# simonfuhrmann/mve

Measured on NVIDIA H100. Metric: mvs_depth_pixels_per_second, higher is better.
Workload: dtype f32

## Files before the change

### mve_b200/csrc/b200mvs.cu

```cuda
#include "../../include/b200mvs.h"
#include "patch_opt.cuh"
#include "patch_warp.cuh"
#include "patch_thread.cuh"
#include "pset_device.cuh"
#include "device_buffer.cuh"
#include "plan_device.cuh"

#include <algorithm>
#include <cmath>
#include <cstdarg>
#include <cstddef>
#include <cstdio>
#include <cstring>
#include <cstdlib>
#include <functional>
#include <map>
#include <chrono>
#include <ctime>
#include <mutex>
#include <string>
#include <thread>
#include <atomic>
#include <vector>

// ... 619 lines not shown
}

__host__ __device__ inline int slots_to_ids(const int* gview, int n_global, unsigned word, int32_t ids[4])
{
    int n = 0;
#pragma unroll
    for (int k = 0; k < 4; ++k) {
        const unsigned sl = (word >> (8 * k)) & 0xFF;
        ids[k] = sl < (unsigned)n_global ? gview[sl] : -1;
        n += ids[k] >= 0;
    }
    return n;
}

__global__ void k_slots_to_ids(const JobParams job, int32_t* __restrict__ out, bool aligned16)
{
    const size_t p = (size_t)blockIdx.x * blockDim.x + threadIdx.x;
    if (p >= (size_t)job.W * job.H) return;
    int32_t ids[4];
    slots_to_ids(job.gview, job.n_global, __ldg(job.slots + p), ids);
    int32_t* o = out + 4 * p;
    if (aligned16) *reinterpret_cast<int4*>(o) = make_int4(ids[0], ids[1], ids[2], ids[3]);
    else { o[0] = ids[0]; o[1] = ids[1]; o[2] = ids[2]; o[3] = ids[3]; }
}

#ifndef OPT_MIN_BLOCKS
#define OPT_MIN_BLOCKS 1
#endif
constexpr int OPT_WARPS = OPT_TPB / 32;
using PatchT = b200mvs::PatchW;
using PatchT1 = b200mvs::PatchT;
constexpr size_t OPT_LUT_BYTES = sizeof(float) * (256 * LUT_STRIDE);
constexpr size_t OPT_SMEM_BYTES = OPT_LUT_BYTES + (size_t)OPT_TPB * sizeof(PatchT1) + PatchT1::MT_BYTES;
static_assert(OPT_SMEM_BYTES + 8 + 1024 <= 196 * 1024, "the patch kernels' shared memory must stay within the 196 KB carve-out");
__device__ __forceinline__ PatchT1& thread_patch(float* smem)
{
    return reinterpret_cast<PatchT1*>(reinterpret_cast<unsigned char*>(smem) + OPT_LUT_BYTES)[threadIdx.x];
}

__device__ __forceinline__ Entry load_entry(const Entry* p)
{
    const int4 a = __ldcg(reinterpret_cast<const int4*>(p));
    const int4 b = __ldcg(reinterpret_cast<const int4*>(p) + 1);
    Entry e;
    e.xy = a.x; e.jobdir = a.y; e.conf = __int_as_float(a.z); e.depth = __int_as_float(a.w);
    e.dzI = __int_as_float(b.x); e.dzJ = __int_as_float(b.y); e.slots = (unsigned)b.z; e.pad = b.w;
    return e;
}

__device__ __forceinline__ PatchIn patch_in(const Entry& e)
{
    PatchIn pi;
    pi.x = entry_x(e); pi.y = entry_y(e);
    pi.depth = e.depth; pi.dzI = e.dzI; pi.dzJ = e.dzJ; pi.slots = e.slots;
    return pi;
}

__device__ __forceinline__ unsigned long long global_timer_ns()
{
    unsigned long long t;
    asm volatile("mov.u64 %0, %%globaltimer;" : "=l"(t));
    return t;
}

__device__ __forceinline__ void optimise_entries(PatchT& p, const Entry* list, PatchOut* res, unsigned long long n,
                                                 unsigned long long* ticket, const JobParams* jobs, unsigned long long* counters)
{
// ... 35 lines not shown
            const unsigned long long w = base + (unsigned long long)__popc(act & ((1u << lane) - 1u));
            if (w >= n) break;
            idx = w;
            const Entry e = load_entry(&list[w]);
            p.begin(&jobs[entry_job(e)], patch_in(e));
            have = true;
            ++opts;
        }
        if (p.step()) {
            PatchOut po;
            p.finish(po);
            res[idx] = po;
            have = false;
        }
    }
    if (opts) {
        atomicAdd(&counters[C_SETS], (unsigned long long)p.n_sets);
        atomicAdd(&counters[C_OPTS], (unsigned long long)opts);
        p.n_sets = 0u;
    }
}

#ifndef OPT_THREAD_MIN
#define OPT_THREAD_MIN 8192
#endif

__global__ void __launch_bounds__(OPT_TPB, OPT_MIN_BLOCKS)
k_optimize(const Entry* __restrict__ in, PatchOut* __restrict__ out, int n, int mode,
           const DevSettings* __restrict__ st, const JobParams* __restrict__ jobs, const ViewParams* __restrict__ views,
           const float* __restrict__ g_lut, unsigned long long* counters)
{
    extern __shared__ float smem[];
    for (int i = threadIdx.x; i < 256 * LUT_STRIDE; i += blockDim.x) smem[i] = g_lut[i / LUT_STRIDE];
    __syncthreads();
    if (mode == 2 || (mode == 0 && n >= OPT_THREAD_MIN)) {
        PatchT1& p = thread_patch(smem);
        bind_thread(p, st, views, smem, (int)threadIdx.x);
        optimise_entries_t(p, in, out, (unsigned long long)n, &counters[C_TICKET], jobs, counters);
    } else {
        PatchT p;
        bind_thread(p, st, views, smem, (int)threadIdx.x);
        optimise_entries(p, in, out, (unsigned long long)n, &counters[C_TICKET], jobs, counters);
    }
}

__device__ __forceinline__ unsigned long long entry_key(const Entry& e)
{
    return ((unsigned long long)__float_as_uint(e.conf) << 8) | (unsigned long long)(7 - entry_dir(e));
}

struct FrontierParams {
    Entry* list[2];
    Entry* run;
    Entry* run2;
    unsigned* tile_cnt;
    unsigned long long* tile_off;
    long long n_tiles;
    PatchOut* res;
    unsigned char* written;
    unsigned long long cap;
    int n_seeds, n_jobs;
    const DevSettings* st;
    const JobParams* jobs;
    const ViewParams* views;
    const float* lut;
    unsigned long long* counters;
// ... 135 lines not shown
        const int j = entry_job(e);
        const JobParams& J = P.jobs[j];
        const int x = entry_x(e), y = entry_y(e);
        const int nx[4] = {x - 1, x + 1, x, x};
        const int ny[4] = {y, y, y - 1, y + 1};
#pragma unroll
        for (int d = 0; d < 4; ++d) {
            const float c = __ldcg(&J.conf[ny[d] * J.W + nx[d]]);
            if (c < r.conf - 0.05f || c == 0.f) push_entry(P, 1 - p, child_entry(pack_xy(nx[d], ny[d]), j, d, r));
        }
    }
}

__device__ __forceinline__ bool end_round(FrontierCtl* ctl, unsigned long long n_cur, const HostMirror* host)
{
    ctl->rounds += 1ull;
    if (n_cur > ctl->peak) ctl->peak = n_cur;
    return host->cancel != 0;
}

__global__ void k_frontier_resume(const FrontierParams P)
{
    FrontierCtl* const ctl = P.ctl;
    const size_t gtid = (size_t)blockIdx.x * blockDim.x + threadIdx.x, gthreads = (size_t)gridDim.x * blockDim.x;
    push_neighbours(P, ctl->resume_p, ctl->resume_sorted ? P.run2 : P.run, ctl->resume_nrun, gtid, gthreads);
    if (gtid == 0) ctl->stop = end_round(ctl, ctl->resume_ncur, P.host) ? ST_CANCELLED : ST_RUN;
}

__global__ void __launch_bounds__(OPT_TPB, OPT_MIN_BLOCKS)
k_frontier(const FrontierParams P)
{
    extern __shared__ float smem[];
    for (int i = threadIdx.x; i < 256 * LUT_STRIDE; i += blockDim.x) smem[i] = P.lut[i / LUT_STRIDE];
    __syncthreads();
    const int lane = threadIdx.x & 31;
    const size_t gtid = (size_t)blockIdx.x * blockDim.x + threadIdx.x, gthreads = (size_t)gridDim.x * blockDim.x;
    FrontierCtl* const ctl = P.ctl;
    unsigned long long* const cnt = P.counters;
    unsigned long long* const filled = cnt + C_NUM;
    const bool lead = blockIdx.x == 0 && threadIdx.x == 0;
    const bool thresholded = P.band_bins > 0 || P.topk > 0;
    unsigned long long t_prev = lead ? global_timer_ns() : 0ull;
    unsigned long long n_bar = 0ull;
#define PHASE_END(ph) do { grid_barrier(&ctl->bar); ++n_bar; if (lead) { const unsigned long long t_ = global_timer_ns(); ctl->ns[ph] += t_ - t_prev; t_prev = t_; } } while (0)

    int p = P.first_list;
    bool seed_round = P.n_seeds > 0;
    for (;;) {
        unsigned long long n_cur = seed_round ? (unsigned long long)P.n_seeds : __ldcg(&ctl->nlist[p]);
        if (n_cur > P.cap) n_cur = P.cap;
        if (__ldcg(&ctl->stop) != ST_RUN || n_cur == 0ull) break;
        unsigned long long n_run = n_cur;
        if (!seed_round) {
        Entry* const cur = P.list[p];
        if (blockIdx.x == 0) {
            if (threadIdx.x == 0) { P.host->round = ctl->rounds; P.host->queue = n_cur; }
            for (int j = threadIdx.x; j < P.n_jobs; j += blockDim.x) {
                P.host_filled[j] = __ldcg(&filled[j]);
                if (P.host_cancel_job[j]) P.job_cancel[j] = 1;
            }
        }
        for (size_t i = gtid; i < n_cur; i += gthreads) {
            const Entry e = load_entry(&cur[i]);
            const int j = entry_job(e);
            const JobParams& J = P.jobs[j];
            const int idx = pixel_of(J, e);
// ... 1589 lines not shown
```

### mve_b200/csrc/patch_opt.cuh

```cuda
#pragma once
#if defined(B200MVS_HOST_EMU)
#include "simt_emu.h"
#else
#include <cuda_runtime.h>
#endif
#include <stdint.h>
#include <cstddef>

namespace b200mvs {

constexpr int MAX_LEVELS = 12;
constexpr int MAX_GLOBAL = 32;
constexpr int MAX_LOCAL = 4;
constexpr unsigned FULL = 0xffffffffu;
constexpr int NS = 25;
constexpr int CENTER = 12;
constexpr int LUT_REP = 32;
constexpr int LUT_STRIDE = 64;

struct alignas(16) LevelParams {
    float ax, ay, cx, cy;
    int w, h;
    int pitch;
    int pad;
// ... 211 lines not shown
                              ((stage == POST) & ((p.iter + 1) % 5 == 4));
        float cand[MAX_GLOBAL];
        PassOut po = {0.f, 0.f, 0.f, 0.f, 0.f};
        p.pass(a_cand, a_cs, a_ncc, a_normal, cand, po);
        if (stage == LVS_CTOR || stage == LVS_REPL) {
            p.lvs_greedy(cand);
            if (!p.is(F_LVS_OK)) { if (stage == LVS_CTOR) p.pk &= ~F_OPTI; p.set_stage(DONE); return true; }
            p.set_stage((stage == LVS_CTOR) ? CTOR : REPL);
            return false;
        }
        if (!p.is(F_OPTI)) { p.set_stage(DONE); return true; }
        if (stage == POST) {
            const int n = p.nsel();
            const unsigned dfb = (p.pk >> SH_DF) & ((1u << n) - 1u);
            const unsigned tbr = ((p.iter == 14) ? dfb : 0u) | p.low_ncc_mask();
            if (tbr) {
                p.pk |= F_VIEW_REMOVED;
                p.sel_erase_mask(tbr);
                p.pk &= ~F_LVS_OK;
                p.set_stage(LVS_REPL);
                return false;
            }
            if (dfb == 0u) { p.pk |= F_CONVERGED; p.set_stage(DONE); return true; }
            ++p.iter;
        } else if (stage == REPL) {
            ++p.iter;
        }
        while (p.iter < 4 && p.is(F_OPTI)) {
            const bool moved = depth_step(p, po);
            ++p.iter;
            if (moved && p.is(F_OPTI)) { p.set_stage(FIRST); return false; }
        }
        if (!p.is(F_OPTI)) { p.set_stage(DONE); return true; }
        if (!((unsigned)p.iter < p.st->max_iterations && p.is(F_LVS_OK))) { p.set_stage(DONE); return true; }
        const bool normal = (p.iter % 5 == 4) || p.is(F_VIEW_REMOVED);
        p.put(F_NORMAL, normal);
        if (!p.is(F_HAS_NCC) || (normal && !p.is(F_HAS_NORMAL))) { p.set_stage(PRE); return false; }
        p.pk &= ~F_OPTI;
        if (normal) { normal_step(p, po); p.pk &= ~F_VIEW_REMOVED; p.pk |= F_WAS_NORMAL; }
        else { depth_step(p, po); p.pk &= ~F_WAS_NORMAL; }
        if (!p.is(F_OPTI)) { p.set_stage(DONE); return true; }
        p.set_stage(POST);
        return false;
    }
};

}
```

### mve_b200/csrc/patch_thread.cuh

```cuda
#pragma once
#include "patch_opt.cuh"
#if defined(B200MVS_HOST_EMU)
#include <cassert>
#endif

#ifndef OPT_TPB
#define OPT_TPB 384
#endif

namespace b200mvs {

struct alignas(8) SampleOffset { float di, dj; };
#if !defined(B200MVS_HOST_EMU)
__constant__
#endif
static const SampleOffset k_sample_offset[NS] = {
    {-2.f, -2.f}, {-1.f, -2.f}, {0.f, -2.f}, {1.f, -2.f}, {2.f, -2.f},
    {-2.f, -1.f}, {-1.f, -1.f}, {0.f, -1.f}, {1.f, -1.f}, {2.f, -1.f},
    {-2.f,  0.f}, {-1.f,  0.f}, {0.f,  0.f}, {1.f,  0.f}, {2.f,  0.f},
    {-2.f,  1.f}, {-1.f,  1.f}, {0.f,  1.f}, {1.f,  1.f}, {2.f,  1.f},
    {-2.f,  2.f}, {-1.f,  2.f}, {0.f,  2.f}, {1.f,  2.f}, {2.f,  2.f}};

struct PatchT : PatchState {
    const DevSettings* st;
    const ViewParams* views;
#if defined(B200MVS_HOST_EMU)
    const float* lut_tab;
    unsigned lane4;
    unsigned mt_k[NS];
#endif
    const JobParams* job;
    unsigned xy;
    float u0x, u0y, u0z;
    float uax, uay, uaz;
    float ubx, uby, ubz;
    float c0x, c0y, c0z;
    float mx0, mx1, mx2;
    float crx, cry, crz;
    float cpx, cpy, cpz;
    float mfp, inv_mfp;
    float mm, inv_mm, sqrDevX;
    unsigned selp;
    float cs[MAX_LOCAL][3];
    float ncc[MAX_LOCAL];

    __device__ __forceinline__ int sel(int k) const { return (int)((selp >> (8 * k)) & 0xFFu); }
    __device__ __forceinline__ int px() const { return (int)(xy & 0xFFFFu); }
    __device__ __forceinline__ int py() const { return (int)(xy >> 16); }

    template <typename T> static __device__ __forceinline__ T get4(const T (&a)[MAX_LOCAL], int k)
    {
        return k == 0 ? a[0] : (k == 1 ? a[1] : (k == 2 ? a[2] : a[3]));
    }
    template <typename T> static __device__ __forceinline__ void set4(T (&a)[MAX_LOCAL], int k, T v)
    {
#pragma unroll
        for (int i = 0; i < MAX_LOCAL; ++i) if (i == k) a[i] = v;
    }

    __device__ __forceinline__ unsigned lane_offset() const
    {
#if defined(B200MVS_HOST_EMU)
        return lane4;
#else
        return (threadIdx.x & 31u) << 2;
#endif
    }
    __device__ __forceinline__ const float* table() const
    {
#if defined(B200MVS_HOST_EMU)
        return lut_tab;
#else
        extern __shared__ float b200mvs_dyn_smem[];
        return b200mvs_dyn_smem;
#endif
    }

#if defined(B200MVS_HOST_EMU)
    static constexpr unsigned MT_STRIDE = 1u;
#else
    static constexpr unsigned MT_STRIDE = OPT_TPB;
#endif
    static constexpr size_t MT_BYTES = sizeof(unsigned) * NS * OPT_TPB;
    __device__ __forceinline__ unsigned* mt_tab()
    {
#if defined(B200MVS_HOST_EMU)
        return mt_k;
#else
        extern __shared__ float b200mvs_dyn_smem[];
        return reinterpret_cast<unsigned*>(b200mvs_dyn_smem + (256 * LUT_STRIDE + OPT_TPB * (sizeof(PatchT) / sizeof(float)))) + threadIdx.x;
#endif
    }

    __device__ __forceinline__ void sample_ray(float di, float dj, float& ux, float& uy, float& uz, float& inv) const
    {
        ux = u0x + di * uax + dj * ubx;
        uy = u0y + di * uay + dj * uby;
        uz = u0z + di * uaz + dj * ubz;
        inv = rsqrt_fast(ux * ux + uy * uy + uz * uz);
    }

    __device__ __forceinline__ void compute_points()
    {
        bool bad = false;
#pragma unroll 5
        for (int k = 0; k < NS; ++k) {
            const float t = depth + (float)(k % 5 - 2) * dzI + (float)(k / 5 - 2) * dzJ;
            bad |= t <= 0.f;
        }
        if (bad) pk &= ~F_REF_OK;
        cpx = c0x + depth * crx;
        cpy = c0y + depth * cry;
        cpz = c0z + depth * crz;
        const ViewParams* rv = &views[job->ref_view];
        const float z = __ldg(&rv->w2c[8]) * cpx + __ldg(&rv->w2c[9]) * cpy + __ldg(&rv->w2c[10]) * cpz + __ldg(&rv->w2c[11]);
        mfp = z * job->ki0;
        inv_mfp = rcp_fast(mfp);
    }

    __device__ __forceinline__ void init_sampler(int x, int y)
    {
        const float* const lut_tab = table();
        const unsigned lane4 = lane_offset();
        pk &= ~F_REF_OK; mm = 0.f; inv_mm = 0.f; sqrDevX = 0.f;
        mx0 = mx1 = mx2 = 0.f;
        crx = cry = crz = cpx = cpy = cpz = mfp = inv_mfp = 0.f;
        if (x - 2 < 0 || y - 2 < 0 || x + 2 > job->W - 1 || y + 2 > job->H - 1) return;
        {
            const ViewParams* rv = &views[job->ref_view];
            const float r0 = __ldg(&rv->rot[0]), r1 = __ldg(&rv->rot[1]), r2 = __ldg(&rv->rot[2]), r3 = __ldg(&rv->rot[3]), r4 = __ldg(&rv->rot[4]);
            const float r5 = __ldg(&rv->rot[5]), r6 = __ldg(&rv->rot[6]), r7 = __ldg(&rv->rot[7]), r8 = __ldg(&rv->rot[8]);
            const float vx = job->ki0 * ((float)x + 0.5f) + job->ki2, vy = job->ki4 * ((float)y + 0.5f) + job->ki5;
            u0x = r0 * vx + r3 * vy + r6; u0y = r1 * vx + r4 * vy + r7; u0z = r2 * vx + r5 * vy + r8;
            uax = r0 * job->ki0; uay = r1 * job->ki0; uaz = r2 * job->ki0;
            ubx = r3 * job->ki4; uby = r4 * job->ki4; ubz = r5 * job->ki4;
            c0x = __ldg(&rv->campos[0]); c0y = __ldg(&rv->campos[1]); c0z = __ldg(&rv->campos[2]);
            const float inv = rsqrt_fast(u0x * u0x + u0y * u0y + u0z * u0z);
            crx = u0x * inv; cry = u0y * inv; crz = u0z * inv;
        }
        pk |= F_REF_OK;
        unsigned* const mt = mt_tab();
        const uchar4* row = job->ref_img + (size_t)(y - 2) * job->ref_pitch + (x - 2);
        float s0 = 0.f, s1 = 0.f, s2 = 0.f;
#pragma unroll 1
        for (int j = 0; j < 5; ++j) {
#pragma unroll
            for (int i = 0; i < 5; ++i) {
                const unsigned t = reinterpret_cast<const unsigned*>(row)[i];
                s0 += lut_k<0>(lut_tab, lane4, t); s1 += lut_k<1>(lut_tab, lane4, t); s2 += lut_k<2>(lut_tab, lane4, t);
                mt[(5 * j + i) * MT_STRIDE] = t;
            }
            row += job->ref_pitch;
        }
        mm = (s0 + s1 + s2) / (3.f * NS);
        if (mm < 0.01f || mm > 0.99f) { pk &= ~F_REF_OK; return; }
        inv_mm = 1.f / mm;
        mx0 = (s0 * inv_mm) / (float)NS; mx1 = (s1 * inv_mm) / (float)NS; mx2 = (s2 * inv_mm) / (float)NS;
        float dev = 0.f;
#pragma unroll 1
        for (int j = 0; j < 5; ++j) {
#pragma unroll
            for (int i = 0; i < 5; ++i) {
                const unsigned t = mt[(5 * j + i) * MT_STRIDE];
                const float e0 = lut_k<0>(lut_tab, lane4, t) * inv_mm - mx0, e1 = lut_k<1>(lut_tab, lane4, t) * inv_mm - mx1, e2 = lut_k<2>(lut_tab, lane4, t) * inv_mm - mx2;
                dev += e0 * e0 + e1 * e1 + e2 * e2;
            }
        }
        sqrDevX = dev;
        compute_points();
    }

    struct Staged {
        uint4 Q;
        unsigned mt;
        float fx, fy, gx, gy;
    };
    struct Sweep {
        const float* lut;
        unsigned lane4;
        float inv_mm;
        float u0x, u0y, u0z, uax, uay, uaz, ubx, uby, ubz, depth, dzI, dzJ;
        const unsigned* mt;
        float A0x, A0y, A0z, W0x, W0y, W0z, Wax, Way, Waz, Wbx, Wby, Wbz;
        float Lax, Lay, Lcx, Lcy, wm1, hm1, step, dd;
        const uint4* quad;
        unsigned qpitch;
        float pv0, pv1, pv2;
        float c0, c1, c2;
        bool nrm;
// ... 49 lines not shown
            const float omfx = sub_rn(1.f, fx), omfy = sub_rn(1.f, fy), wxy = fma_rn(fy, gx, mul_rn(fx, gy));
            float n[3], d[3];
#pragma unroll
            for (int ch = 0; ch < 3; ++ch) {
                const float x0 = fma_rn(omfx, a[ch], mul_rn(fx, b[ch]));
                const float x3 = fma_rn(omfx, c[ch], mul_rn(fx, e[ch]));
                n[ch] = fma_rn(omfy, x0, mul_rn(fy, x3));
                const float t = fma_rn(gx, sub_rn(b[ch], a[ch]), mul_rn(gy, sub_rn(c[ch], a[ch])));
                d[ch] = mul_rn(fma_rn(wxy, add_rn(sub_rn(sub_rn(a[ch], b[ch]), c[ch]), e[ch]), t), dd);
            }
            const float y0 = sub_rn(n[0], pv0), y1 = sub_rn(n[1], pv1), y2 = sub_rn(n[2], pv2);
            Sya = add_rn(Sya, y0); Syb = add_rn(Syb, y1); Syc = add_rn(Syc, y2);
            Syya = fma_rn(y0, y0, Syya); Syyb = fma_rn(y1, y1, Syyb); Syyc = fma_rn(y2, y2, Syyc);
            Smya = fma_rn(m[0], y0, Smya); Smyb = fma_rn(m[1], y1, Smyb); Smyc = fma_rn(m[2], y2, Smyc);
            Sdma = fma_rn(d[0], m[0], Sdma); Sdmb = fma_rn(d[1], m[1], Sdmb); Sdmc = fma_rn(d[2], m[2], Sdmc);
            Sdna = fma_rn(d[0], n[0], Sdna); Sdnb = fma_rn(d[1], n[1], Sdnb); Sdnc = fma_rn(d[2], n[2], Sdnc);
            Sdda = fma_rn(d[0], d[0], Sdda); Sddb = fma_rn(d[1], d[1], Sddb); Sddc = fma_rn(d[2], d[2], Sddc);
            if (nrm) {
                const float di = k_sample_offset[k].di, dj = k_sample_offset[k].dj;
                const float g0 = mul_rn(c0, d[0]), g1 = mul_rn(c1, d[1]), g2 = mul_rn(c2, d[2]);
                const float q = fma_rn(g2, g2, fma_rn(g0, g0, mul_rn(g1, g1)));
                const float s = fma_rn(g2, fma_rn(-c2, n[2], m[2]), fma_rn(g0, fma_rn(-c0, n[0], m[0]), mul_rn(g1, fma_rn(-c1, n[1], m[1]))));
                const float qi = mul_rn(di, q), qj = mul_rn(dj, q);
                A1 = add_rn(A1, qi); A2 = add_rn(A2, qj); A3 = fma_rn(di, qi, A3); A4 = fma_rn(dj, qi, A4); A5 = fma_rn(dj, qj, A5);
                B1 = fma_rn(di, s, B1); B2 = fma_rn(dj, s, B2);
            }
        }
    };

    __device__ __forceinline__ void pass(bool candidates, bool cs_pending, bool want_ncc, bool want_normal, float* cand, PassOut& po)
    {
        const float* const lut_tab = table();
        const unsigned lane4 = lane_offset();
        const float u0x = this->u0x, u0y = this->u0y, u0z = this->u0z, uax = this->uax, uay = this->uay, uaz = this->uaz;
        const float ubx = this->ubx, uby = this->uby, ubz = this->ubz;
        const float depth = this->depth, dzI = this->dzI, dzJ = this->dzJ;
        const float inv_mm = this->inv_mm;
        const JobParams* const job = this->job;
        float num = 0.f, den = 0.f;
        double D0 = 0.0, D1 = 0.0, D2 = 0.0, D3 = 0.0, D4 = 0.0, D5 = 0.0, E0 = 0.0, E1 = 0.0, E2 = 0.0;
        bool cs_active = cs_pending && st->use_color_scale;
        if (!candidates) pk &= want_ncc ? ~((0xFFu << SH_COL) | (0xFu << SH_DF)) : ~(0xFFu << SH_COL);
        const int count = candidates ? job->n_global : nsel();
        const float pv0 = mx0 * mm, pv1 = mx1 * mm, pv2 = mx2 * mm;
#pragma unroll 1
        for (int k = 0; k < count; ++k) {
            int slot = k;
            if (candidates) { if (!((avail >> k) & 1u)) continue; }
            else slot = sel(k);
            const ViewParams* V = &views[job->gview[slot]];
            ++n_sets;
            float c0 = 1.f, c1 = 1.f, c2 = 1.f;
            if (!candidates) {
                c0 = k == 0 ? cs[0][0] : (k == 1 ? cs[1][0] : (k == 2 ? cs[2][0] : cs[3][0]));
                c1 = k == 0 ? cs[0][1] : (k == 1 ? cs[1][1] : (k == 2 ? cs[2][1] : cs[3][1]));
                c2 = k == 0 ? cs[0][2] : (k == 1 ? cs[1][2] : (k == 2 ? cs[2][2] : cs[3][2]));
            }
            unsigned r = 0u;
            float A0x = 0.f, A0y = 0.f, A0z = 0.f, W0x = 0.f, W0y = 0.f, W0z = 0.f, Wax = 0.f, Way = 0.f, Waz = 0.f, Wbx = 0.f, Wby = 0.f, Wbz = 0.f;
            float Lax = 0.f, Lay = 0.f, Lcx = 0.f, Lcy = 0.f, wm1 = 0.f, hm1 = 0.f, dd = 0.f, step = 0.f;
            int Lpitch = 0;
            const uint4* Lquad = nullptr;
            {
                const float4 wa = __ldg(reinterpret_cast<const float4*>(&V->w2c[0]));
                const float4 wb = __ldg(reinterpret_cast<const float4*>(&V->w2c[4]));
                const float4 wc = __ldg(reinterpret_cast<const float4*>(&V->w2c[8]));
                A0x = wa.x * c0x + wa.y * c0y + wa.z * c0z + wa.w;
                A0y = wb.x * c0x + wb.y * c0y + wb.z * c0z + wb.w;
                A0z = wc.x * c0x + wc.y * c0y + wc.z * c0z + wc.w;
                W0x = wa.x * u0x + wa.y * u0y + wa.z * u0z; W0y = wb.x * u0x + wb.y * u0y + wb.z * u0z; W0z = wc.x * u0x + wc.y * u0y + wc.z * u0z;
                Wax = wa.x * uax + wa.y * uay + wa.z * uaz; Way = wb.x * uax + wb.y * uay + wb.z * uaz; Waz = wc.x * uax + wc.y * uay + wc.z * uaz;
                Wbx = wa.x * ubx + wa.y * uby + wa.z * ubz; Wby = wb.x * ubx + wb.y * uby + wb.z * ubz; Wbz = wc.x * ubx + wc.y * uby + wc.z * ubz;
                const float nz = wc.x * cpx + wc.y * cpy + wc.z * cpz + wc.w;
                const float nfp = nz * __ldg(&V->inv_ax0);
                if (mfp > 0.f && !(nfp <= 0.f)) {
                    const int l = level_of(V, nfp, inv_mfp);
                    const float4 kk = __ldg(reinterpret_cast<const float4*>(&V->lv[l].ax));
                    const int4 g = __ldg(reinterpret_cast<const int4*>(&V->lv[l].w));
                    Lax = kk.x; Lay = kk.y; Lcx = kk.z; Lcy = kk.w; wm1 = (float)(g.x - 1); hm1 = (float)(g.y - 1); Lpitch = g.z;
                    Lquad = reinterpret_cast<const uint4*>(__ldg(reinterpret_cast<const unsigned long long*>(&V->lv[l].quad)));
                    const float inv0 = rsqrt_fast(u0x * u0x + u0y * u0y + u0z * u0z);
                    const float sa = depth * inv0, sb = (depth + 1.f) * inv0;
                    const float hz1 = A0z + sa * W0z, hz2 = A0z + sb * W0z;
                    const float i1 = rcp_fast(hz1), i2 = rcp_fast(hz2);
                    const float ddx = (Lax * (A0x + sb * W0x) + Lcx * hz2) * i2 - (Lax * (A0x + sa * W0x) + Lcx * hz1) * i1;
                    const float ddy = (Lay * (A0y + sb * W0y) + Lcy * hz2) * i2 - (Lay * (A0y + sa * W0y) + Lcy * hz1) * i1;
                    const float dd2 = ddx * ddx + ddy * ddy;
                    dd = dd2 * rsqrt_fast(dd2);
                    step = rcp_fast(dd);
                    r = dd > 0.f ? 3u : 1u;
                }
            }
            const bool need_ncc = candidates || want_ncc;
            const bool cs_view = !candidates && cs_active;
            float nccv = -1.f;
#pragma unroll 1
            for (int rep = 0; rep < 2 && r != 0u; ++rep) {
                const bool second = rep == 1;
                if (second && !(cs_view && want_normal && (r & 2u))) break;
                const bool gn = !candidates && (r & 2u) && (second || !(cs_view && want_normal));
                const bool nrm = gn && want_normal;
                Sweep sw;
                sw.lut = lut_tab; sw.lane4 = lane4; sw.inv_mm = inv_mm;
                sw.u0x = u0x; sw.u0y = u0y; sw.u0z = u0z; sw.uax = uax; sw.uay = uay; sw.uaz = uaz; sw.ubx = ubx; sw.uby = uby; sw.ubz = ubz;
                sw.mt = mt_tab();
                sw.depth = depth; sw.dzI = dzI; sw.dzJ = dzJ;
                sw.A0x = A0x; sw.A0y = A0y; sw.A0z = A0z; sw.W0x = W0x; sw.W0y = W0y; sw.W0z = W0z;
                sw.Wax = Wax; sw.Way = Way; sw.Waz = Waz; sw.Wbx = Wbx; sw.Wby = Wby; sw.Wbz = Wbz;
                sw.Lax = Lax; sw.Lay = Lay; sw.Lcx = Lcx; sw.Lcy = Lcy; sw.wm1 = wm1; sw.hm1 = hm1; sw.step = step; sw.dd = dd;
// ... 24 lines not shown
                    const float sqrDevY = (Syya - Sya * Sya * inv_n) + (Syyb - Syb * Syb * inv_n) + (Syyc - Syc * Syc * inv_n);
                    const float Sen = (Smya - mx0 * Sya) + (Smyb - mx1 * Syb) + (Smyc - mx2 * Syc);
                    const float p = sqrDevX * sqrDevY;
                    nccv = p > 0.f ? Sen * rsqrt_fast(p) : -1.f;
                }
                if (!second && cs_view) {
                    const float Mna = Smya + pv0 * ((float)NS * mx0), Mnb = Smyb + pv1 * ((float)NS * mx1), Mnc = Smyc + pv2 * ((float)NS * mx2);
                    const float Nna = Syya + pv0 * (2.f * Sya + (float)NS * pv0), Nnb = Syyb + pv1 * (2.f * Syb + (float)NS * pv1);
                    const float Nnc = Syyc + pv2 * (2.f * Syc + (float)NS * pv2);
                    float cc[3] = {c0, c1, c2};
                    const float ab[3] = {Mna - c0 * Nna, Mnb - c1 * Nnb, Mnc - c2 * Nnc};
                    const float aa[3] = {Nna, Nnb, Nnc};
                    colour_scale_step(cc, ab, aa);
                    c0 = cc[0]; c1 = cc[1]; c2 = cc[2];
#pragma unroll
                    for (int i = 0; i < MAX_LOCAL; ++i) if (i == k) { cs[i][0] = c0; cs[i][1] = c1; cs[i][2] = c2; }
                }
                if (gn) {
                    const float vn = c0 * (Sdma - c0 * Sdna) + c1 * (Sdmb - c1 * Sdnb) + c2 * (Sdmc - c2 * Sdnc);
                    const float vd = c0 * c0 * Sdda + c1 * c1 * Sddb + c2 * c2 * Sddc;
                    num += vn; den += vd;
                    if (nrm) {
                        D0 += (double)vd; D1 += (double)A1; D2 += (double)A2; D3 += (double)A3; D4 += (double)A4; D5 += (double)A5;
                        E0 += (double)vn; E1 += (double)B1; E2 += (double)B2;
                    }
                }
            }
            if (!candidates) {
                if (r & 1u) pk |= 1u << (SH_COL + k);
                if (r & 2u) pk |= 1u << (SH_DER + k);
                if (cs_active && !(r & 1u)) cs_active = false;
                if (want_ncc) {
                    const float v = (r & 1u) ? nccv : -1.f;
                    if (fabsf(v - get4(ncc, k)) > st->min_refine_diff) pk |= 1u << (SH_DF + k);
                    set4(ncc, k, v);
                }
            } else {
                const float v = (r & 1u) ? nccv : -1.f;
                if (v < st->min_ncc) avail &= ~(1u << k);
                else cand[k] = v;
            }
        }
        if (candidates) return;
        po.num = num; po.den = den;
        put(F_HAS_NORMAL, want_normal);
        put(F_HAS_NCC, want_ncc);
        if (want_normal) {
            const double m[9] = {D0, D1, D2, D1, D3, D4, D2, D4, D5};
            const double det = m[0] * m[4] * m[8] + m[1] * m[5] * m[6] + m[2] * m[3] * m[7]
                             - m[2] * m[4] * m[6] - m[1] * m[3] * m[8] - m[0] * m[5] * m[7];
            put(F_SINGULAR, det == 0.0);
            double inv[9];
            inv[0] = m[4] * m[8] - m[5] * m[7];
            inv[1] = m[2] * m[7] - m[1] * m[8];
            inv[2] = m[1] * m[5] - m[2] * m[4];
            inv[3] = m[5] * m[6] - m[3] * m[8];
            inv[4] = m[0] * m[8] - m[2] * m[6];
            inv[5] = m[2] * m[3] - m[0] * m[5];
            inv[6] = m[3] * m[7] - m[4] * m[6];
            inv[7] = m[1] * m[6] - m[0] * m[7];
            inv[8] = m[0] * m[4] - m[1] * m[3];
#pragma unroll
            for (int q = 0; q < 9; ++q) inv[q] /= det;
            po.nX0 = (float)(inv[0] * E0 + inv[1] * E1 + inv[2] * E2);
            po.nX1 = (float)(inv[3] * E0 + inv[4] * E1 + inv[5] * E2);
            po.nX2 = (float)(inv[6] * E0 + inv[7] * E1 + inv[8] * E2);
        }
    }

    __device__ __forceinline__ void sel_erase_mask(unsigned mask)
    {
        const int n = nsel();
// ... 2 lines not shown
#pragma unroll
        for (int k = 0; k < MAX_LOCAL; ++k) {
            if (k < n && !((mask >> k) & 1u)) {
                const unsigned s8 = (selp >> (8 * k)) & 0xFFu;
                const float a = cs[k][0], b = cs[k][1], c = cs[k][2], v = ncc[k];
                packed = (packed & ~(0xFFu << (8 * cnt))) | (s8 << (8 * cnt));
#pragma unroll
                for (int q = 0; q < MAX_LOCAL; ++q) if (q == cnt) { cs[q][0] = a; cs[q][1] = b; cs[q][2] = c; ncc[q] = v; }
                ++cnt;
            }
        }
        selp = packed;
        set_nsel(cnt);
    }
    __device__ __forceinline__ void sel_insert(int slot, float cs_init)
    {
        const int n = nsel();
        int pos = 0;
#pragma unroll
        for (int k = 0; k < MAX_LOCAL; ++k) if (k < n && sel(k) < slot) ++pos;
#pragma unroll
        for (int q = MAX_LOCAL - 1; q > 0; --q)
            if (q > pos && q <= n) { cs[q][0] = cs[q - 1][0]; cs[q][1] = cs[q - 1][1]; cs[q][2] = cs[q - 1][2]; ncc[q] = ncc[q - 1]; }
#pragma unroll
        for (int q = 0; q < MAX_LOCAL; ++q) if (q == pos) { cs[q][0] = cs[q][1] = cs[q][2] = cs_init; ncc[q] = 0.f; }
        const unsigned low = pos == 0 ? 0u : (selp & (0xFFFFFFFFu >> (32 - 8 * pos)));
        const unsigned high = pos >= 3 ? 0u : ((selp >> (8 * pos)) << (8 * (pos + 1)));
        selp = low | ((unsigned)slot << (8 * pos)) | high;
        set_nsel(n + 1);
    }

    __device__ __forceinline__ void lvs_greedy(const float* cand)
    {
        const unsigned N = st->nr_recon_neighbors;
        const float cs_init = 1.f / mm;
        float rdx = cpx - c0x, rdy = cpy - c0y, rdz = cpz - c0z;
        {
            const float nn = sqrtf(rdx * rdx + rdy * rdy + rdz * rdz);
            rdx /= nn; rdy /= nn; rdz /= nn;
        }
        const int G = job->n_global;
        bool found = true;
        while ((unsigned)nsel() < N && found) {
            found = false;
            float maxScore = 0.f;
            int maxView = 0;
#pragma unroll 1
            for (int c = 0; c < G; ++c) {
                if (!((avail >> c) & 1u)) continue;
                float vdx, vdy, vdz, epx, epy, epz, nfp;
                view_geometry(&views[job->gview[c]], cpx, cpy, cpz, rdx, rdy, rdz, vdx, vdy, vdz, epx, epy, epz, nfp);
                float score = cand[c];
                if (mfp / nfp < 0.5f) score *= 0.01f;
                float dp = clamp1(rdx * vdx + rdy * vdy + rdz * vdz);
                score *= plx_weight(deg_acos(dp));
                const int ns = nsel();
#pragma unroll 1
                for (int k = 0; k < ns; ++k) {
                    float sx, sy, sz, ex, ey, ez, sfp;
                    view_geometry(&views[job->gview[sel(k)]], cpx, cpy, cpz, rdx, rdy, rdz, sx, sy, sz, ex, ey, ez, sfp);
                    lvs_weigh(score, vdx, vdy, vdz, epx, epy, epz, sx, sy, sz, ex, ey, ez, st->min_parallax);
                }
                if (score > maxScore) { maxScore = score; maxView = c; found = true; }
            }
            if (found) {
                sel_insert(maxView, cs_init);
                avail &= ~(1u << maxView);
            }
        }
        if ((unsigned)nsel() == N) pk |= F_LVS_OK;
    }

    __device__ __forceinline__ void begin(const JobParams* j, const PatchIn& in)
    {
        job = j;
        xy = ((unsigned)in.x & 0xFFFFu) | ((unsigned)in.y << 16);
        reset(in);
        u0x = u0y = u0z = uax = uay = uaz = ubx = uby = ubz = c0x = c0y = c0z = 0.f;
        init_sampler(in.x, in.y);
        selp = in.slots;
        int n = 0;
#pragma unroll
        for (int k = 0; k < MAX_LOCAL; ++k) {
            if (sel(k) != 0xFF) n = k + 1;
            cs[k][0] = cs[k][1] = cs[k][2] = 0.f; ncc[k] = 0.f;
        }
        set_nsel(n);
        if (!is(F_REF_OK)) { pk &= ~F_OPTI; return; }
        const unsigned N = st->nr_recon_neighbors;
        if ((unsigned)n == N) pk |= F_LVS_OK;
        else if ((unsigned)n > N) {
            n = 0;
            set_nsel(0);
            selp = 0xFFFFFFFFu;
        }
        avail = job->n_global >= 32 ? FULL : ((1u << job->n_global) - 1u);
#pragma unroll
        for (int k = 0; k < MAX_LOCAL; ++k) if (k < n) avail &= ~(1u << sel(k));
        const float ci = 1.f / mm;
#pragma unroll
        for (int k = 0; k < MAX_LOCAL; ++k) { cs[k][0] = cs[k][1] = cs[k][2] = ci; }
        set_stage(is(F_LVS_OK) ? CTOR : LVS_CTOR);
    }

    __device__ __forceinline__ unsigned low_ncc_mask() const
    {
        const int n = nsel();
        unsigned m = 0u;
#pragma unroll
        for (int k = 0; k < MAX_LOCAL; ++k)
            if (k < n && ncc[k] < st->accept_ncc) m |= 1u << k;
        return m;
    }

    __device__ __forceinline__ bool step() { return auto_step(*this); }

    __device__ __forceinline__ void finish(PatchOut& out)
    {
        finish_state(out);
        const int n = nsel();
        out.slots = n >= 4 ? selp : (selp | (0xFFFFFFFFu << (8 * n)));
        if (!is(F_CONVERGED)) return;
        float mean = 0.f;
#pragma unroll
        for (int k = 0; k < MAX_LOCAL; ++k) if (k < n) mean += ncc[k];
        mean /= (float)n;
        float px[4], py[4], pz[4];
        const float di_[4] = {2.f, -2.f, 0.f, 0.f}, dj_[4] = {0.f, 0.f, -2.f, 2.f};
#pragma unroll
        for (int q = 0; q < 4; ++q) {
            float ux, uy, uz, inv;
            sample_ray(di_[q], dj_[q], ux, uy, uz, inv);
            const float s1 = (depth + di_[q] * dzI + dj_[q] * dzJ) * inv;
            px[q] = c0x + s1 * ux; py[q] = c0y + s1 * uy; pz[q] = c0z + s1 * uz;
        }
        const float ax_ = px[0] - px[1], ay_ = py[0] - py[1], az_ = pz[0] - pz[1];
        const float bx_ = px[2] - px[3], by_ = py[2] - py[3], bz_ = pz[2] - pz[3];
        confidence(out, ax_, ay_, az_, bx_, by_, bz_, crx, cry, crz, mean, st->accept_ncc);
    }
};

#if !defined(B200MVS_HOST_EMU)
static_assert(sizeof(PatchT) % 16 == 8, "PatchT stride in shared memory must be 8 mod 16 bytes");
#endif

__device__ __forceinline__ void bind_thread(PatchT& p, const DevSettings* st, const ViewParams* views, const float* lut_rep, int tid)
{
    p.st = st; p.views = views;
#if defined(B200MVS_HOST_EMU)
    p.lut_tab = lut_rep; p.lane4 = 4u * (unsigned)(tid & (LUT_REP - 1));
#else
    (void)lut_rep; (void)tid;
#endif
    p.pk = (unsigned)PatchT::DONE << PatchT::SH_STAGE;
    p.n_sets = 0u;
}

}
```

### mve_b200/csrc/patch_warp.cuh

```cuda
#pragma once
#include "patch_opt.cuh"

namespace b200mvs {

__device__ __forceinline__ float warp_sum(float v)
{
#pragma unroll
    for (int o = 16; o > 0; o >>= 1) v += __shfl_xor_sync(FULL, v, o);
    return v;
}
__device__ __forceinline__ double warp_sum(double v)
{
#pragma unroll
    for (int o = 16; o > 0; o >>= 1) v += __shfl_xor_sync(FULL, v, o);
    return v;
}
__device__ __forceinline__ float warp_max(float v)
{
#pragma unroll
    for (int o = 16; o > 0; o >>= 1) v = fmaxf(v, __shfl_xor_sync(FULL, v, o));
    return v;
}

__device__ __forceinline__ void warp_sum4(int lane, float& a, float& b, float& c, float& d)
// ... 16 lines not shown
    const bool h16 = lane & 16;
    float k = h16 ? b : a;
    const float s = h16 ? a : b;
    k += __shfl_xor_sync(FULL, s, 16);
    k += __shfl_xor_sync(FULL, k, 8);
    k += __shfl_xor_sync(FULL, k, 4);
    k += __shfl_xor_sync(FULL, k, 2);
    k += __shfl_xor_sync(FULL, k, 1);
    a = __shfl_sync(FULL, k, 0); b = __shfl_sync(FULL, k, 16);
}

struct PatchW : PatchState {
    const DevSettings* st;
    const JobParams* job;
    const ViewParams* views;
    const ViewParams* rv;
    const float* lut_tab;
    unsigned lane4;
    int lane;
    bool act;
    float fi, fj;
    float rx, ry, rz;
    float px, py, pz;
    float m0, m1, m2;
    float e0, e1, e2;
    float crx, cry, crz;
    float cpx, cpy, cpz;
    float mfp, inv_mfp;
    float mm, sqrDevX;
    int sel_l;
    float cs0_l, cs1_l, cs2_l;
    float ncc_l;
    float cand_ncc_l;

    __device__ __forceinline__ void project(const float (&w)[12], const LevelParams& L, float X, float Y, float Z,
                                            float& x, float& y) const
    {
        const float c0 = w[0] * X + w[1] * Y + w[2] * Z + w[3];
        const float c1 = w[4] * X + w[5] * Y + w[6] * Z + w[7];
        const float c2 = w[8] * X + w[9] * Y + w[10] * Z + w[11];
        const float ic2 = rcp_fast(c2);
        x = (L.ax * c0 + L.cx * c2) * ic2 - 0.5f;
        y = (L.ay * c1 + L.cy * c2) * ic2 - 0.5f;
    }

    __device__ __forceinline__ void compute_points()
    {
        const float t = depth + fi * dzI + fj * dzJ;
        const bool bad = act && (t <= 0.f);
        if (__any_sync(FULL, bad)) pk &= ~F_REF_OK;
        px = __ldg(&rv->campos[0]) + t * rx;
        py = __ldg(&rv->campos[1]) + t * ry;
        pz = __ldg(&rv->campos[2]) + t * rz;
        cpx = __shfl_sync(FULL, px, CENTER);
        cpy = __shfl_sync(FULL, py, CENTER);
        cpz = __shfl_sync(FULL, pz, CENTER);
        const float z = __ldg(&rv->w2c[8]) * cpx + __ldg(&rv->w2c[9]) * cpy + __ldg(&rv->w2c[10]) * cpz + __ldg(&rv->w2c[11]);
        mfp = z * job->ki0;
        inv_mfp = rcp_fast(mfp);
    }

    __device__ __forceinline__ void init_sampler(int x, int y)
    {
        act = lane < NS;
        const int di = act ? (lane % 5) - 2 : 0, dj = act ? (lane / 5) - 2 : 0;
        fi = (float)di; fj = (float)dj;
// ... 330 lines not shown
```

Baseline: 70.62 million.

## Shrink per-thread patch state by recomputing derived rays and sharing launch pointers

Removes many cached fields (ray step vectors, centre direction/point, inverse mfp/mm, xy, settings/views pointers) from the shared-memory PatchT struct and recomputes them on demand. The settings and views pointers now live in a single block-wide shared struct written by thread 0. The smaller struct is meant to cut shared-memory footprint per block, and the carve-out assertion is tightened to 164 KB so more blocks can be resident. In exchange there are extra rsqrt/rcp/FMA and global loads at each use site.

After: 71.86 million (median of 6 runs). +1.8%, better.

```diff
diff --git a/mve_b200/csrc/b200mvs.cu b/mve_b200/csrc/b200mvs.cu
--- a/mve_b200/csrc/b200mvs.cu
+++ b/mve_b200/csrc/b200mvs.cu
@@ -675,7 +675,8 @@
 using PatchT1 = b200mvs::PatchT;
 constexpr size_t OPT_LUT_BYTES = sizeof(float) * (256 * LUT_STRIDE);
 constexpr size_t OPT_SMEM_BYTES = OPT_LUT_BYTES + (size_t)OPT_TPB * sizeof(PatchT1) + PatchT1::MT_BYTES;
-static_assert(OPT_SMEM_BYTES + 8 + 1024 <= 196 * 1024, "the patch kernels' shared memory must stay within the 196 KB carve-out");
+constexpr size_t OPT_STATIC_SMEM_BYTES = 32;
+static_assert(OPT_SMEM_BYTES + OPT_STATIC_SMEM_BYTES + 1024 <= 164 * 1024, "the patch kernels' shared memory must stay within the 164 KB carve-out");
 __device__ __forceinline__ PatchT1& thread_patch(float* smem)
 {
     return reinterpret_cast<PatchT1*>(reinterpret_cast<unsigned char*>(smem) + OPT_LUT_BYTES)[threadIdx.x];
@@ -777,6 +778,7 @@
 {
     extern __shared__ float smem[];
     for (int i = threadIdx.x; i < 256 * LUT_STRIDE; i += blockDim.x) smem[i] = g_lut[i / LUT_STRIDE];
+    bind_launch(st, views);
     __syncthreads();
     if (mode == 2 || (mode == 0 && n >= OPT_THREAD_MIN)) {
         PatchT1& p = thread_patch(smem);
@@ -978,6 +980,7 @@
 {
     extern __shared__ float smem[];
     for (int i = threadIdx.x; i < 256 * LUT_STRIDE; i += blockDim.x) smem[i] = P.lut[i / LUT_STRIDE];
+    bind_launch(P.st, P.views);
     __syncthreads();
     const int lane = threadIdx.x & 31;
     const size_t gtid = (size_t)blockIdx.x * blockDim.x + threadIdx.x, gthreads = (size_t)gridDim.x * blockDim.x;
diff --git a/mve_b200/csrc/patch_opt.cuh b/mve_b200/csrc/patch_opt.cuh
--- a/mve_b200/csrc/patch_opt.cuh
+++ b/mve_b200/csrc/patch_opt.cuh
@@ -267,7 +267,7 @@
             if (moved && p.is(F_OPTI)) { p.set_stage(FIRST); return false; }
         }
         if (!p.is(F_OPTI)) { p.set_stage(DONE); return true; }
-        if (!((unsigned)p.iter < p.st->max_iterations && p.is(F_LVS_OK))) { p.set_stage(DONE); return true; }
+        if (!((unsigned)p.iter < p.settings()->max_iterations && p.is(F_LVS_OK))) { p.set_stage(DONE); return true; }
         const bool normal = (p.iter % 5 == 4) || p.is(F_VIEW_REMOVED);
         p.put(F_NORMAL, normal);
         if (!p.is(F_HAS_NCC) || (normal && !p.is(F_HAS_NORMAL))) { p.set_stage(PRE); return false; }
diff --git a/mve_b200/csrc/patch_thread.cuh b/mve_b200/csrc/patch_thread.cuh
--- a/mve_b200/csrc/patch_thread.cuh
+++ b/mve_b200/csrc/patch_thread.cuh
@@ -21,32 +21,66 @@
     {-2.f,  1.f}, {-1.f,  1.f}, {0.f,  1.f}, {1.f,  1.f}, {2.f,  1.f},
     {-2.f,  2.f}, {-1.f,  2.f}, {0.f,  2.f}, {1.f,  2.f}, {2.f,  2.f}};
 
+#if !defined(B200MVS_HOST_EMU)
+struct ThreadLaunch { const DevSettings* st; const ViewParams* views; };
+__shared__ ThreadLaunch thread_launch;
+#endif
+
 struct PatchT : PatchState {
+    unsigned selp;
+    const JobParams* job;
+    float u0x, u0y, u0z;
+    float mx0, mx1, mx2;
+    float c0x, c0y, c0z;
+    float mfp;
+    float mm, sqrDevX;
+    float cs[MAX_LOCAL][3];
+    float ncc[MAX_LOCAL];
+#if defined(B200MVS_HOST_EMU)
     const DevSettings* st;
     const ViewParams* views;
-#if defined(B200MVS_HOST_EMU)
     const float* lut_tab;
     unsigned lane4;
     unsigned mt_k[NS];
 #endif
-    const JobParams* job;
-    unsigned xy;
-    float u0x, u0y, u0z;
-    float uax, uay, uaz;
-    float ubx, uby, ubz;
-    float c0x, c0y, c0z;
-    float mx0, mx1, mx2;
-    float crx, cry, crz;
-    float cpx, cpy, cpz;
-    float mfp, inv_mfp;
-    float mm, inv_mm, sqrDevX;
-    unsigned selp;
-    float cs[MAX_LOCAL][3];
-    float ncc[MAX_LOCAL];
 
     __device__ __forceinline__ int sel(int k) const { return (int)((selp >> (8 * k)) & 0xFFu); }
-    __device__ __forceinline__ int px() const { return (int)(xy & 0xFFFFu); }
-    __device__ __forceinline__ int py() const { return (int)(xy >> 16); }
+    __device__ __forceinline__ const DevSettings* settings() const
+    {
+#if defined(B200MVS_HOST_EMU)
+        return st;
+#else
+        return thread_launch.st;
+#endif
+    }
+    __device__ __forceinline__ const ViewParams* view(int v) const
+    {
+#if defined(B200MVS_HOST_EMU)
+        return &views[v];
+#else
+        return &thread_launch.views[v];
+#endif
+    }
+    __device__ __forceinline__ const ViewParams* ref_view() const { return view(job->ref_view); }
+
+    __device__ __forceinline__ void ray_steps(float& uax, float& uay, float& uaz, float& ubx, float& uby, float& ubz) const
+    {
+        const ViewParams* rv = ref_view();
+        const float ki0 = job->ki0, ki4 = job->ki4;
+        uax = mul_rn(__ldg(&rv->rot[0]), ki0); uay = mul_rn(__ldg(&rv->rot[1]), ki0); uaz = mul_rn(__ldg(&rv->rot[2]), ki0);
+        ubx = mul_rn(__ldg(&rv->rot[3]), ki4); uby = mul_rn(__ldg(&rv->rot[4]), ki4); ubz = mul_rn(__ldg(&rv->rot[5]), ki4);
+    }
+    __device__ __forceinline__ void centre_dir(float& crx, float& cry, float& crz) const
+    {
+        const float inv = rsqrt_fast(fma_rn(u0z, u0z, fma_rn(u0x, u0x, mul_rn(u0y, u0y))));
+        crx = mul_rn(u0x, inv); cry = mul_rn(u0y, inv); crz = mul_rn(u0z, inv);
+    }
+    __device__ __forceinline__ void centre_point(float& cpx, float& cpy, float& cpz) const
+    {
+        float crx, cry, crz;
+        centre_dir(crx, cry, crz);
+        cpx = fma_rn(depth, crx, c0x); cpy = fma_rn(depth, cry, c0y); cpz = fma_rn(depth, crz, c0z);
+    }
 
     template <typename T> static __device__ __forceinline__ T get4(const T (&a)[MAX_LOCAL], int k)
     {
@@ -90,14 +124,6 @@
         extern __shared__ float b200mvs_dyn_smem[];
         return reinterpret_cast<unsigned*>(b200mvs_dyn_smem + (256 * LUT_STRIDE + OPT_TPB * (sizeof(PatchT) / sizeof(float)))) + threadIdx.x;
 #endif
-    }
-
-    __device__ __forceinline__ void sample_ray(float di, float dj, float& ux, float& uy, float& uz, float& inv) const
-    {
-        ux = u0x + di * uax + dj * ubx;
-        uy = u0y + di * uay + dj * uby;
-        uz = u0z + di * uaz + dj * ubz;
-        inv = rsqrt_fast(ux * ux + uy * uy + uz * uz);
     }
 
     __device__ __forceinline__ void compute_points()
@@ -109,34 +135,28 @@
             bad |= t <= 0.f;
         }
         if (bad) pk &= ~F_REF_OK;
-        cpx = c0x + depth * crx;
-        cpy = c0y + depth * cry;
-        cpz = c0z + depth * crz;
-        const ViewParams* rv = &views[job->ref_view];
+        const ViewParams* rv = ref_view();
+        float cpx, cpy, cpz;
+        centre_point(cpx, cpy, cpz);
         const float z = __ldg(&rv->w2c[8]) * cpx + __ldg(&rv->w2c[9]) * cpy + __ldg(&rv->w2c[10]) * cpz + __ldg(&rv->w2c[11]);
         mfp = z * job->ki0;
-        inv_mfp = rcp_fast(mfp);
     }
 
     __device__ __forceinline__ void init_sampler(int x, int y)
     {
         const float* const lut_tab = table();
         const unsigned lane4 = lane_offset();
-        pk &= ~F_REF_OK; mm = 0.f; inv_mm = 0.f; sqrDevX = 0.f;
+        pk &= ~F_REF_OK; mm = 0.f; sqrDevX = 0.f;
         mx0 = mx1 = mx2 = 0.f;
-        crx = cry = crz = cpx = cpy = cpz = mfp = inv_mfp = 0.f;
+        c0x = c0y = c0z = mfp = 0.f;
         if (x - 2 < 0 || y - 2 < 0 || x + 2 > job->W - 1 || y + 2 > job->H - 1) return;
         {
-            const ViewParams* rv = &views[job->ref_view];
+            const ViewParams* rv = ref_view();
             const float r0 = __ldg(&rv->rot[0]), r1 = __ldg(&rv->rot[1]), r2 = __ldg(&rv->rot[2]), r3 = __ldg(&rv->rot[3]), r4 = __ldg(&rv->rot[4]);
             const float r5 = __ldg(&rv->rot[5]), r6 = __ldg(&rv->rot[6]), r7 = __ldg(&rv->rot[7]), r8 = __ldg(&rv->rot[8]);
             const float vx = job->ki0 * ((float)x + 0.5f) + job->ki2, vy = job->ki4 * ((float)y + 0.5f) + job->ki5;
             u0x = r0 * vx + r3 * vy + r6; u0y = r1 * vx + r4 * vy + r7; u0z = r2 * vx + r5 * vy + r8;
-            uax = r0 * job->ki0; uay = r1 * job->ki0; uaz = r2 * job->ki0;
-            ubx = r3 * job->ki4; uby = r4 * job->ki4; ubz = r5 * job->ki4;
             c0x = __ldg(&rv->campos[0]); c0y = __ldg(&rv->campos[1]); c0z = __ldg(&rv->campos[2]);
-            const float inv = rsqrt_fast(u0x * u0x + u0y * u0y + u0z * u0z);
-            crx = u0x * inv; cry = u0y * inv; crz = u0z * inv;
         }
         pk |= F_REF_OK;
         unsigned* const mt = mt_tab();
@@ -154,7 +174,7 @@
         }
         mm = (s0 + s1 + s2) / (3.f * NS);
         if (mm < 0.01f || mm > 0.99f) { pk &= ~F_REF_OK; return; }
-        inv_mm = 1.f / mm;
+        const float inv_mm = 1.f / mm;
         mx0 = (s0 * inv_mm) / (float)NS; mx1 = (s1 * inv_mm) / (float)NS; mx2 = (s2 * inv_mm) / (float)NS;
         float dev = 0.f;
 #pragma unroll 1
@@ -270,14 +290,15 @@
     {
         const float* const lut_tab = table();
         const unsigned lane4 = lane_offset();
-        const float u0x = this->u0x, u0y = this->u0y, u0z = this->u0z, uax = this->uax, uay = this->uay, uaz = this->uaz;
-        const float ubx = this->ubx, uby = this->uby, ubz = this->ubz;
+        const float u0x = this->u0x, u0y = this->u0y, u0z = this->u0z;
+        float uax, uay, uaz, ubx, uby, ubz;
+        ray_steps(uax, uay, uaz, ubx, uby, ubz);
         const float depth = this->depth, dzI = this->dzI, dzJ = this->dzJ;
-        const float inv_mm = this->inv_mm;
+        const float inv_mm = 1.f / mm;
         const JobParams* const job = this->job;
         float num = 0.f, den = 0.f;
         double D0 = 0.0, D1 = 0.0, D2 = 0.0, D3 = 0.0, D4 = 0.0, D5 = 0.0, E0 = 0.0, E1 = 0.0, E2 = 0.0;
-        bool cs_active = cs_pending && st->use_color_scale;
+        bool cs_active = cs_pending && settings()->use_color_scale;
         if (!candidates) pk &= want_ncc ? ~((0xFFu << SH_COL) | (0xFu << SH_DF)) : ~(0xFFu << SH_COL);
         const int count = candidates ? job->n_global : nsel();
         const float pv0 = mx0 * mm, pv1 = mx1 * mm, pv2 = mx2 * mm;
@@ -286,7 +307,7 @@
             int slot = k;
             if (candidates) { if (!((avail >> k) & 1u)) continue; }
             else slot = sel(k);
-            const ViewParams* V = &views[job->gview[slot]];
+            const ViewParams* V = view(job->gview[slot]);
             ++n_sets;
             float c0 = 1.f, c1 = 1.f, c2 = 1.f;
             if (!candidates) {
@@ -300,6 +321,8 @@
             int Lpitch = 0;
             const uint4* Lquad = nullptr;
             {
+                float cpx, cpy, cpz;
+                centre_point(cpx, cpy, cpz);
                 const float4 wa = __ldg(reinterpret_cast<const float4*>(&V->w2c[0]));
                 const float4 wb = __ldg(reinterpret_cast<const float4*>(&V->w2c[4]));
                 const float4 wc = __ldg(reinterpret_cast<const float4*>(&V->w2c[8]));
@@ -312,7 +335,7 @@
                 const float nz = wc.x * cpx + wc.y * cpy + wc.z * cpz + wc.w;
                 const float nfp = nz * __ldg(&V->inv_ax0);
                 if (mfp > 0.f && !(nfp <= 0.f)) {
-                    const int l = level_of(V, nfp, inv_mfp);
+                    const int l = level_of(V, nfp, rcp_fast(mfp));
                     const float4 kk = __ldg(reinterpret_cast<const float4*>(&V->lv[l].ax));
                     const int4 g = __ldg(reinterpret_cast<const int4*>(&V->lv[l].w));
                     Lax = kk.x; Lay = kk.y; Lcx = kk.z; Lcy = kk.w; wm1 = (float)(g.x - 1); hm1 = (float)(g.y - 1); Lpitch = g.z;
@@ -403,12 +426,12 @@
                 if (cs_active && !(r & 1u)) cs_active = false;
                 if (want_ncc) {
                     const float v = (r & 1u) ? nccv : -1.f;
-                    if (fabsf(v - get4(ncc, k)) > st->min_refine_diff) pk |= 1u << (SH_DF + k);
+                    if (fabsf(v - get4(ncc, k)) > settings()->min_refine_diff) pk |= 1u << (SH_DF + k);
                     set4(ncc, k, v);
                 }
             } else {
                 const float v = (r & 1u) ? nccv : -1.f;
-                if (v < st->min_ncc) avail &= ~(1u << k);
+                if (v < settings()->min_ncc) avail &= ~(1u << k);
                 else cand[k] = v;
             }
         }
@@ -477,8 +500,11 @@
 
     __device__ __forceinline__ void lvs_greedy(const float* cand)
     {
+        const DevSettings* const st = settings();
         const unsigned N = st->nr_recon_neighbors;
         const float cs_init = 1.f / mm;
+        float cpx, cpy, cpz;
+        centre_point(cpx, cpy, cpz);
         float rdx = cpx - c0x, rdy = cpy - c0y, rdz = cpz - c0z;
         {
             const float nn = sqrtf(rdx * rdx + rdy * rdy + rdz * rdz);
@@ -494,7 +520,7 @@
             for (int c = 0; c < G; ++c) {
                 if (!((avail >> c) & 1u)) continue;
                 float vdx, vdy, vdz, epx, epy, epz, nfp;
-                view_geometry(&views[job->gview[c]], cpx, cpy, cpz, rdx, rdy, rdz, vdx, vdy, vdz, epx, epy, epz, nfp);
+                view_geometry(view(job->gview[c]), cpx, cpy, cpz, rdx, rdy, rdz, vdx, vdy, vdz, epx, epy, epz, nfp);
                 float score = cand[c];
                 if (mfp / nfp < 0.5f) score *= 0.01f;
                 float dp = clamp1(rdx * vdx + rdy * vdy + rdz * vdz);
@@ -503,7 +529,7 @@
 #pragma unroll 1
                 for (int k = 0; k < ns; ++k) {
                     float sx, sy, sz, ex, ey, ez, sfp;
-                    view_geometry(&views[job->gview[sel(k)]], cpx, cpy, cpz, rdx, rdy, rdz, sx, sy, sz, ex, ey, ez, sfp);
+                    view_geometry(view(job->gview[sel(k)]), cpx, cpy, cpz, rdx, rdy, rdz, sx, sy, sz, ex, ey, ez, sfp);
                     lvs_weigh(score, vdx, vdy, vdz, epx, epy, epz, sx, sy, sz, ex, ey, ez, st->min_parallax);
                 }
                 if (score > maxScore) { maxScore = score; maxView = c; found = true; }
@@ -519,9 +545,8 @@
     __device__ __forceinline__ void begin(const JobParams* j, const PatchIn& in)
     {
         job = j;
-        xy = ((unsigned)in.x & 0xFFFFu) | ((unsigned)in.y << 16);
         reset(in);
-        u0x = u0y = u0z = uax = uay = uaz = ubx = uby = ubz = c0x = c0y = c0z = 0.f;
+        u0x = u0y = u0z = 0.f;
         init_sampler(in.x, in.y);
         selp = in.slots;
         int n = 0;
@@ -532,7 +557,7 @@
         }
         set_nsel(n);
         if (!is(F_REF_OK)) { pk &= ~F_OPTI; return; }
-        const unsigned N = st->nr_recon_neighbors;
+        const unsigned N = settings()->nr_recon_neighbors;
         if ((unsigned)n == N) pk |= F_LVS_OK;
         else if ((unsigned)n > N) {
             n = 0;
@@ -554,7 +579,7 @@
         unsigned m = 0u;
 #pragma unroll
         for (int k = 0; k < MAX_LOCAL; ++k)
-            if (k < n && ncc[k] < st->accept_ncc) m |= 1u << k;
+            if (k < n && ncc[k] < settings()->accept_ncc) m |= 1u << k;
         return m;
     }
 
@@ -572,16 +597,22 @@
         mean /= (float)n;
         float px[4], py[4], pz[4];
         const float di_[4] = {2.f, -2.f, 0.f, 0.f}, dj_[4] = {0.f, 0.f, -2.f, 2.f};
+        float uax, uay, uaz, ubx, uby, ubz;
+        ray_steps(uax, uay, uaz, ubx, uby, ubz);
 #pragma unroll
         for (int q = 0; q < 4; ++q) {
-            float ux, uy, uz, inv;
-            sample_ray(di_[q], dj_[q], ux, uy, uz, inv);
+            const float ux = u0x + di_[q] * uax + dj_[q] * ubx;
+            const float uy = u0y + di_[q] * uay + dj_[q] * uby;
+            const float uz = u0z + di_[q] * uaz + dj_[q] * ubz;
+            const float inv = rsqrt_fast(ux * ux + uy * uy + uz * uz);
             const float s1 = (depth + di_[q] * dzI + dj_[q] * dzJ) * inv;
             px[q] = c0x + s1 * ux; py[q] = c0y + s1 * uy; pz[q] = c0z + s1 * uz;
         }
         const float ax_ = px[0] - px[1], ay_ = py[0] - py[1], az_ = pz[0] - pz[1];
         const float bx_ = px[2] - px[3], by_ = py[2] - py[3], bz_ = pz[2] - pz[3];
-        confidence(out, ax_, ay_, az_, bx_, by_, bz_, crx, cry, crz, mean, st->accept_ncc);
+        float crx, cry, crz;
+        centre_dir(crx, cry, crz);
+        confidence(out, ax_, ay_, az_, bx_, by_, bz_, crx, cry, crz, mean, settings()->accept_ncc);
     }
 };
 
@@ -589,12 +620,22 @@
 static_assert(sizeof(PatchT) % 16 == 8, "PatchT stride in shared memory must be 8 mod 16 bytes");
 #endif
 
+__device__ __forceinline__ void bind_launch(const DevSettings* st, const ViewParams* views)
+{
+#if !defined(B200MVS_HOST_EMU)
+    if (threadIdx.x == 0) { thread_launch.st = st; thread_launch.views = views; }
+#else
+    (void)st; (void)views;
+#endif
+}
+
 __device__ __forceinline__ void bind_thread(PatchT& p, const DevSettings* st, const ViewParams* views, const float* lut_rep, int tid)
 {
+#if defined(B200MVS_HOST_EMU)
     p.st = st; p.views = views;
-#if defined(B200MVS_HOST_EMU)
     p.lut_tab = lut_rep; p.lane4 = 4u * (unsigned)(tid & (LUT_REP - 1));
 #else
+    (void)st; (void)views;
     (void)lut_rep; (void)tid;
 #endif
     p.pk = (unsigned)PatchT::DONE << PatchT::SH_STAGE;
diff --git a/mve_b200/csrc/patch_warp.cuh b/mve_b200/csrc/patch_warp.cuh
--- a/mve_b200/csrc/patch_warp.cuh
+++ b/mve_b200/csrc/patch_warp.cuh
@@ -72,6 +72,8 @@
     float cs0_l, cs1_l, cs2_l;
     float ncc_l;
     float cand_ncc_l;
+
+    __device__ __forceinline__ const DevSettings* settings() const { return st; }
 
     __device__ __forceinline__ void project(const float (&w)[12], const LevelParams& L, float X, float Y, float Z,
                                             float& x, float& y) const
```
